# DoHoonKim8/halo2-lasso

Hardware: AMD Instinct MI355X
Metric: lasso_prove_time_ms (lower is better)
Workload: dtype u256 (BN254 Fr/Fq, 8x u32 Montgomery); 1 GPU; 2^24 AND Lasso lookup (32-bit operands, 4 chunks of 8+8 bits); lookups_per_proof=16777216, pcs=multilinear KZG (BN254), proof_bytes=64256, parallelism=1 GPU

## Files before the change

### bindings/rust/src/sys.rs

```rust
#![allow(non_camel_case_types, dead_code)]
use halo2_curves::bn256::{Fr, G1Affine, G2Affine};
use std::os::raw::{c_char, c_int, c_void};

pub type lh_status = c_int;
pub const LH_OK: lh_status = 0;
pub const LH_ERR_INVALID_SUMCHECK: lh_status = -1;
pub const LH_ERR_INVALID_PCS_PARAM: lh_status = -2;
pub const LH_ERR_INVALID_PCS_OPEN: lh_status = -3;
pub const LH_ERR_INVALID_SNARK: lh_status = -4;
pub const LH_ERR_SERIALIZATION: lh_status = -5;
pub const LH_ERR_TRANSCRIPT: lh_status = -6;
pub const LH_ERR_DEVICE: lh_status = -7;
pub const LH_ERR_ARG: lh_status = -8;

pub const LH_SC_MAX_TERMS: usize = 48;
pub const LH_SC_MAX_FACTORS: usize = 4;
pub const LH_SC_EVALUATIONS: c_int = 0;
pub const LH_SC_COEFFICIENTS: c_int = 1;
pub const LH_LASSO_MAX_CHUNKS: usize = 8;
pub const LH_LASSO_MAX_MEMORIES: usize = 16;
pub const LH_LASSO_MAX_TERMS: usize = 16;
pub const LH_RCCL_UNIQUE_ID_BYTES: usize = 128;

#[repr(C)] pub struct lh_ctx { _p: [u8; 0] }
// ... 159 lines not shown

#[repr(C)]
#[derive(Clone, Copy, Debug, Default)]
pub struct lh_lasso_route {
    pub open_small_depth: u32,
    pub open_small_passes: u32,
    pub eq_factored_rounds: u32,
    pub standard_rounds: u32,
    pub rw_leaf_rounds: u32,
    pub resident_tails: u32,
    pub resident_rounds: u32,
    pub packed_ts_pairs: u32,
    pub derived_commitments: u32,
    pub sorted_dim_reuse: u32,
    pub sharded_rounds: u32,
    pub shard_exchanges: u32,
    pub window_table_jobs: u32,
    pub open_precommit: u32,
    pub resident_layers: u32,
    pub pp_folds: u32,
    pub msm_half_batches: u32,
    pub open_shared_sums: u32,
    pub open_precommit_staged: u32,
    pub reserved: [u32; 5],
}

extern "C" {
    pub fn lh_last_error() -> *const c_char;
    pub fn lh_version() -> *const c_char;
    pub fn lh_ctx_create(device_id: c_int, out: *mut *mut lh_ctx) -> lh_status;
    pub fn lh_ctx_destroy(ctx: *mut lh_ctx);
    pub fn lh_ctx_sync(ctx: *mut lh_ctx) -> lh_status;
    pub fn lh_ctx_stream(ctx: *mut lh_ctx) -> *mut c_void;
    pub fn lh_alloc(ctx: *mut lh_ctx, bytes: usize, d_out: *mut *mut c_void) -> lh_status;
    pub fn lh_free(ctx: *mut lh_ctx, d_ptr: *mut c_void) -> lh_status;
    pub fn lh_upload(ctx: *mut lh_ctx, d_dst: *mut c_void, src: *const c_void, bytes: usize) -> lh_status;
    pub fn lh_download(ctx: *mut lh_ctx, dst: *mut c_void, d_src: *const c_void, bytes: usize) -> lh_status;
    pub fn lh_fr_from_u64(ctx: *mut lh_ctx, d_in: *const u64, n: usize, d_out: *mut Fr) -> lh_status;
    pub fn lh_fr_from_u32(ctx: *mut lh_ctx, d_in: *const u32, n: usize, d_out: *mut Fr) -> lh_status;
    pub fn lh_fr_batch_invert(ctx: *mut lh_ctx, d_in: *const Fr, n: usize, d_out: *mut Fr) -> lh_status;
    pub fn lh_fix_var(ctx: *mut lh_ctx, d_in: *const Fr, n_in: usize, x: *const Fr, d_out: *mut Fr) -> lh_status;
    pub fn lh_eq_xy(ctx: *mut lh_ctx, y: *const Fr, num_vars: usize, d_out: *mut Fr) -> lh_status;
    pub fn lh_evaluate(ctx: *mut lh_ctx, d_polys: *const *const Fr, num_polys: usize, num_vars: usize,
                       point: *const Fr, out_evals: *mut Fr) -> lh_status;
    pub fn lh_lincomb(ctx: *mut lh_ctx, d_polys: *const *const Fr, w: *const Fr, num_polys: usize, n: usize,
                      d_out: *mut Fr) -> lh_status;
    pub fn lh_sumcheck_prove(ctx: *mut lh_ctx, prover_kind: c_int, num_vars: usize, expr: *const lh_sop,
// ... 61 lines not shown
                                      t: *mut lh_transcript) -> lh_status;
    pub fn lh_hyperplonk_verify(vp: *const lh_mkzg_vp, hvp: *const lh_hp_vparam, instances: *const *const Fr,
                                t: *mut lh_transcript) -> lh_status;
    pub fn lh_hyperplonk_verify_phases(vp: *const lh_mkzg_vp, hvp: *const lh_hp_vparam, num_phases: usize,
                                       num_witness_polys: *const usize, num_challenges: *const usize,
                                       instances: *const *const Fr, t: *mut lh_transcript) -> lh_status;
    pub fn lh_hyperplonk_prove_phases_zeromorph(ctx: *mut lh_ctx, srs: *const core::ffi::c_void, poly_size: usize,
                                                pp: *const lh_hp_param, num_phases: usize,
                                                num_witness_polys: *const usize, num_challenges: *const usize,
                                                instances: *const *const Fr, circuit: *const lh_hp_circuit,
                                                t: *mut lh_transcript) -> lh_status;
    pub fn lh_hyperplonk_verify_phases_zeromorph(vp: *const core::ffi::c_void, hvp: *const lh_hp_vparam, num_phases: usize,
                                                 num_witness_polys: *const usize, num_challenges: *const usize,
                                                 instances: *const *const Fr, t: *mut lh_transcript) -> lh_status;
    pub fn lh_debug_jit_source(code: *const u32, num_instrs: usize, num_regs: u32, result_reg: u32, degree: i32,
                               out: *mut core::ffi::c_char, cap: usize, len: *mut usize) -> lh_status;
    pub fn lh_debug_sort_pairs(ctx: *mut lh_ctx, key_bytes: i32, slabs: *const lh_debug_sort_slab, count: usize) -> lh_status;
    pub fn lh_debug_lasso_counters(ctx: *mut lh_ctx, d_dims: *const *const u32, num_cols: usize, n: usize, m: usize,
                                   d_read_ts: *const *mut u32, d_final_cts: *const *mut u32,
                                   d_keep_sorted: *const *mut u32, d_keep_index: *const *mut u32) -> lh_status;
    pub fn lh_debug_sort_plan(n: usize, bits: u32, key_bytes: i32, passes: *mut u32, rb: *mut u32,
                              temp_bytes: *mut usize) -> lh_status;
    pub fn lh_debug_u32_columns(ctx: *mut lh_ctx, op: i32, args: *const lh_debug_u32_args) -> lh_status;
    pub fn lh_ukzg_batch_commit(ctx: *mut lh_ctx, srs: *const c_void, poly_size: usize, d_polys: *const *const Fr,
                                lens: *const usize, num_polys: usize, out_comms: *mut G1Affine) -> lh_status;
    pub fn lh_ukzg_open(ctx: *mut lh_ctx, srs: *const c_void, poly_size: usize, d_poly: *const Fr, len: usize,
                        point: *const Fr, t: *mut lh_transcript) -> lh_status;
    pub fn lh_ukzg_batch_open(ctx: *mut lh_ctx, srs: *const c_void, poly_size: usize, d_polys: *const *const Fr,
                              lens: *const usize, num_polys: usize, points: *const Fr, num_points: usize,
                              evals: *const lh_evaluation, num_evals: usize, t: *mut lh_transcript) -> lh_status;
    pub fn lh_ukzg_vp_setup(s: *const Fr, out: *mut *mut c_void) -> lh_status;
    pub fn lh_ukzg_vp_free(vp: *mut c_void);
    pub fn lh_ukzg_verify(vp: *const c_void, comm: *const G1Affine, point: *const Fr, eval: *const Fr,
                          t: *mut lh_transcript) -> lh_status;
    pub fn lh_ukzg_batch_verify(vp: *const c_void, comms: *const G1Affine, num_comms: usize, points: *const Fr,
                                num_points: usize, evals: *const lh_evaluation, num_evals: usize,
                                t: *mut lh_transcript) -> lh_status;
    pub fn lh_gemini_batch_commit(ctx: *mut lh_ctx, srs: *const c_void, poly_size: usize, d_polys: *const *const Fr,
                                  num_polys: usize, num_vars: usize, out_comms: *mut G1Affine) -> lh_status;
    pub fn lh_gemini_open(ctx: *mut lh_ctx, srs: *const c_void, poly_size: usize, d_poly: *const Fr, num_vars: usize,
                          point: *const Fr, t: *mut lh_transcript) -> lh_status;
    pub fn lh_gemini_batch_open(ctx: *mut lh_ctx, srs: *const c_void, poly_size: usize, num_vars: usize,
                                d_polys: *const *const Fr, num_polys: usize, points: *const Fr, num_points: usize,
                                evals: *const lh_evaluation, num_evals: usize, t: *mut lh_transcript) -> lh_status;
    pub fn lh_gemini_verify(vp: *const c_void, comm: *const G1Affine, point: *const Fr, num_vars: usize, eval: *const Fr,
                            t: *mut lh_transcript) -> lh_status;
// ... 142 lines not shown
```

### halo2-lasso_amd/__init__.py

```python
import ctypes as C

from . import _ffi
from ._ffi import (lh_fr, lh_g1, lh_sop, lh_evaluation, lh_lasso_table, lh_transcript,
                   LH_SC_EVALUATIONS, LH_SC_COEFFICIENTS)

R_MOD = 0x30644E72E131A029B85045B68181585D2833E84879B9709143E1F593F0000001
Q_MOD = 0x30644E72E131A029B85045B68181585D97816A916871CA8D3C208C16D87CFD47
_MONT = 1 << 256
_MONT_INV_R = pow(_MONT, -1, R_MOD)
_MONT_INV_Q = pow(_MONT, -1, Q_MOD)

SUBTABLE_IDENTITY, SUBTABLE_AND, SUBTABLE_XOR = 0, 1, 2
SUBTABLE_OR, SUBTABLE_EQ, SUBTABLE_LTU = 3, 4, 5


class Error(Exception):
    code = None


class InvalidSumcheck(Error):
    code = _ffi.LH_ERR_INVALID_SUMCHECK


class InvalidPcsParam(Error):
# ... 1386 lines not shown
    n_local = (1 << poly.num_vars) >> rho
    out = poly.ctx.alloc(32 * n_local)
    _check(poly.ctx.lib.lh_shard_extract(poly.ctx.h, poly.ptr, n_local, shard_bit, rho, rank, 32, out.ptr))
    return MultilinearPolynomial(poly.ctx, out, poly.num_vars - rho)


def lasso_prove_sharded(pp, table, num_vars, dims_local, transcript):
    if len(dims_local) != table.c:
        raise ArgumentError("expected %d dim columns" % table.c)
    t = table.to_c()
    _check(pp.ctx.lib.lh_lasso_prove_sharded(pp.ctx.h, pp.h, C.byref(t), num_vars, _ptr_array(dims_local), transcript.p))


def lasso_last_timing(ctx):
    out = (C.c_double * _ffi.LH_LASSO_NUM_PHASES)()
    _check(ctx.lib.lh_lasso_last_timing(ctx.h, out))
    names = ["witness", "commit", "surge", "leaves", "gkr", "evals", "open_n", "open_l", "total"]
    return dict(zip(names, list(out)))


ROUTE_FIELDS = ["open_small_depth", "open_small_passes", "eq_factored_rounds", "standard_rounds", "rw_leaf_rounds",
                "resident_tails", "resident_rounds", "packed_ts_pairs", "derived_commitments", "sorted_dim_reuse",
                "sharded_rounds", "shard_exchanges", "window_table_jobs", "open_precommit", "resident_layers", "pp_folds", "msm_half_batches",
                "open_shared_sums", "open_precommit_staged"]


def lasso_last_route(ctx):
    out = (C.c_uint32 * 24)()
    _check(ctx.lib.lh_lasso_last_route(ctx.h, out))
    return dict(zip(ROUTE_FIELDS, [int(v) for v in out]))


def set_option(ctx, name, value):
    _check(ctx.lib.lh_ctx_set_option(ctx.h, name.encode(), int(value)))


def get_option(ctx, name):
    out = C.c_int64(0)
    _check(ctx.lib.lh_ctx_get_option(ctx.h, name.encode(), C.byref(out)))
    return int(out.value)


def profile_enable(ctx, on=True):
    _check(ctx.lib.lh_profile_enable(ctx.h, int(on)))


def profile_read(ctx):
# ... 9 lines not shown
```

### halo2-lasso_amd/_ffi.py

```python
import ctypes as C
import os

_HERE = os.path.dirname(os.path.abspath(__file__))
LIB_PATH = os.path.join(_HERE, "liblasso_hip.so")

LH_OK = 0
LH_ERR_INVALID_SUMCHECK, LH_ERR_INVALID_PCS_PARAM, LH_ERR_INVALID_PCS_OPEN = -1, -2, -3
LH_ERR_INVALID_SNARK, LH_ERR_SERIALIZATION, LH_ERR_TRANSCRIPT, LH_ERR_DEVICE, LH_ERR_ARG = -4, -5, -6, -7, -8
LH_SC_EVALUATIONS, LH_SC_COEFFICIENTS = 0, 1
LH_SC_MAX_TERMS, LH_SC_MAX_FACTORS = 48, 4
LH_LASSO_MAX_CHUNKS, LH_LASSO_MAX_MEMORIES, LH_LASSO_MAX_TERMS = 8, 16, 16
LH_SUBTABLE_IDENTITY, LH_SUBTABLE_AND, LH_SUBTABLE_XOR, LH_SUBTABLE_OR, LH_SUBTABLE_EQ, LH_SUBTABLE_LTU = 0, 1, 2, 3, 4, 5
LH_LASSO_NUM_PHASES = 9
LH_BD_COLUMN_FR, LH_BD_COLUMN_U32 = 0, 1


class lh_fr(C.Structure):
    _fields_ = [("l", C.c_uint64 * 4)]


class lh_g1(C.Structure):
    _fields_ = [("x", C.c_uint64 * 4), ("y", C.c_uint64 * 4)]


# ... 258 lines not shown
                                      C.POINTER(lh_evaluation), _SZ, C.POINTER(lh_transcript)]),
    "lh_g1_axpy": (C.c_int, [_P, _P, _P, _SZ, C.POINTER(lh_fr), _P]),
    "lh_g1_rows_msm": (C.c_int, [_P, _P, C.c_int, C.c_uint32, _SZ, _SZ, _P, C.POINTER(lh_g1)]),
    "lh_hyrax_setup": (C.c_int, [_P, _SZ, _SZ, C.POINTER(_P)]),
    "lh_hyrax_dims": (C.c_int, [_SZ, _SZ, C.POINTER(_SZ), C.POINTER(_SZ), C.POINTER(_SZ)]),
    "lh_hyrax_trim": (C.c_int, [_P, _SZ, _SZ, C.POINTER(_SZ), C.POINTER(_SZ)]),
    "lh_hyrax_batch_commit": (C.c_int, [_P, _P, _SZ, _SZ, C.POINTER(_P), _SZ, _SZ, C.POINTER(lh_g1)]),
    "lh_hyrax_open": (C.c_int, [_P, _P, _SZ, _SZ, _P, _SZ, C.POINTER(lh_fr), C.POINTER(lh_transcript)]),
    "lh_hyrax_batch_open": (C.c_int, [_P, _P, _SZ, _SZ, _SZ, C.POINTER(_P), _SZ, C.POINTER(lh_fr), _SZ,
                                      C.POINTER(lh_evaluation), _SZ, C.POINTER(lh_transcript)]),
    "lh_hyrax_verify": (C.c_int, [_P, _SZ, _SZ, C.POINTER(lh_g1), C.POINTER(lh_fr), _SZ, C.POINTER(lh_fr),
                                  C.POINTER(lh_transcript)]),
    "lh_hyrax_batch_verify": (C.c_int, [_P, _SZ, _SZ, _SZ, C.POINTER(lh_g1), _SZ, C.POINTER(lh_fr), _SZ,
                                        C.POINTER(lh_evaluation), _SZ, C.POINTER(lh_transcript)]),
    "lh_debug_jit_source": (C.c_int, [C.POINTER(C.c_uint32), _SZ, C.c_uint32, C.c_uint32, C.c_int, C.c_char_p, _SZ,
                                      C.POINTER(_SZ)]),
    "lh_debug_sort_pairs": (C.c_int, [_P, C.c_int, C.POINTER(lh_debug_sort_slab), _SZ]),
    "lh_debug_lasso_counters": (C.c_int, [_P, C.POINTER(_P), _SZ, _SZ, _SZ, C.POINTER(_P), C.POINTER(_P), C.POINTER(_P),
                                          C.POINTER(_P)]),
    "lh_debug_sort_plan": (C.c_int, [_SZ, C.c_uint, C.c_int, C.POINTER(C.c_uint), C.POINTER(C.c_uint), C.POINTER(_SZ)]),
    "lh_debug_msm_plan": (C.c_int, [_SZ, C.POINTER(_SZ), C.POINTER(C.c_uint32), C.POINTER(C.c_uint32), C.c_int, C.c_int,
                                    C.POINTER(C.c_uint64), C.POINTER(_SZ)]),
    "lh_debug_u32_columns": (C.c_int, [_P, C.c_int, C.POINTER(lh_debug_u32_args)]),
    "lh_keccak_transcript_hash_io": (C.c_int, [C.POINTER(lh_transcript), C.POINTER(lh_hash_transcript)]),
    "lh_brakedown_setup": (C.c_int, [_P, _SZ, C.c_int, C.c_char_p, C.POINTER(_P)]),
    "lh_brakedown_derive": (C.c_int, [_SZ, C.c_int, C.POINTER(_P)]),
    "lh_brakedown_param_info": (C.c_int, [_P, C.POINTER(_SZ), C.POINTER(_SZ), C.POINTER(_SZ), C.POINTER(_SZ),
                                          C.POINTER(_SZ)]),
    "lh_brakedown_trim": (C.c_int, [_P, _SZ]),
    "lh_brakedown_param_free": (None, [_P]),
    "lh_brakedown_encode": (C.c_int, [_P, C.POINTER(lh_fr), C.POINTER(lh_fr)]),
    "lh_brakedown_commit": (C.c_int, [_P, _P, _P, _SZ, C.POINTER(_P)]),
    "lh_brakedown_batch_commit": (C.c_int, [_P, _P, C.POINTER(_P), _SZ, _SZ, C.POINTER(_P)]),
    "lh_brakedown_commit_columns": (C.c_int, [_P, _P, C.POINTER(_P), C.POINTER(C.c_int), C.POINTER(_SZ), _SZ, C.POINTER(_P)]),
    "lh_brakedown_comm_root": (C.c_int, [_P, C.c_char_p]),
    "lh_brakedown_comm_rows": (C.c_int, [_P, _P, _P]),
    "lh_brakedown_comm_rows_device": (C.c_int, [_P, C.POINTER(_P)]),
    "lh_brakedown_comm_tree": (C.c_int, [_P, _P, C.c_char_p]),
    "lh_brakedown_comm_stage": (C.c_int, [_P, _P, _P, _P]),
    "lh_brakedown_comm_free": (None, [_P]),
    "lh_hyperplonk_prove_brakedown": (C.c_int, [_P, _P, C.POINTER(lh_hp_param), C.POINTER(_P), C.POINTER(_P),
                                                C.POINTER(C.POINTER(lh_fr)), C.POINTER(_P), C.POINTER(lh_transcript),
                                                C.POINTER(lh_hash_transcript)]),
    "lh_hyperplonk_prove_phases_brakedown": (C.c_int, [_P, _P, C.POINTER(lh_hp_param), C.POINTER(_P), C.POINTER(_P), _SZ,
                                                       C.POINTER(_SZ), C.POINTER(_SZ), C.POINTER(C.POINTER(lh_fr)),
                                                       C.POINTER(lh_hp_circuit), C.POINTER(lh_transcript),
# ... 67 lines not shown
```

### halo2-lasso_amd/csrc/capi.cpp

```cpp
#include "host.hpp"
#include "brakedown.hpp"
#include <memory>

using namespace lh;

struct lh_ctx {
  Ctx c;
};
struct lh_srs {
  Srs s;
};
struct lh_mkzg_vp {
  VerifierParams* p;
};
struct lh_usrs {
  USrs s;
};
struct lh_zm_vp {
  ZmVerifierParams* p;
};
struct lh_ukzg_vp {
  UkzgVerifierParams* p;
};
struct lh_ipa_param {
// ... 2119 lines not shown
    case LH_U32_QUAD_SUMS: k_quad_sums(c, cols, a->lens, a->count, dw, a->n, (Fr*)a->d_out); break;
    case LH_U32_LINCOMB_MIXED:
      k_lincomb_mixed(c, (const Fr* const*)a->d_fr, (const Fr*)a->w_fr, a->num_fr, cols, a->lens, (const Fr*)a->w, a->count, a->n,
                      (Fr*)a->d_out);
      break;
    case LH_U32_LINCOMB_FOLD_SMALL:
      *a->taken = k_lincomb_fold_small(c, cols, a->lens, (const Fr*)a->w, a->count, a->n, r0, (Fr*)a->d_out) ? 1 : 0;
      break;
    default: {
      Fr* two = (Fr*)c.pin(65536) + 1024;
      if (op == LH_U32_LINCOMB_BIND2) {
        k_lincomb_bind2(c, cols, a->lens, (const Fr*)a->w, a->count, r0, r1, dw, a->n, (Fr*)a->d_out, two);
        memcpy(a->out_host, two, 64);
      } else {
        k_sc_round_u32_bind2(c, cols[0], dw, r0, r1, a->n, (Fr*)a->d_out, two);
        memcpy(a->out_host, two, 32);
      }
    }
  }
  c.sync();
  LH_CATCH
}

lh_status lh_profile_enable(lh_ctx* ctx, int on) {
  LH_TRY NEED_CTX(ctx);
  ctx->c.sync();
  ctx->c.prof = on == 1;
  ctx->c.prof_recs.clear();
  std::vector<ProfRec> drop;
  ctx->c.live_resolve(drop);
  ctx->c.live = on == 2;
  if (ctx->c.helper) {
    ctx->c.helper->live_resolve(drop);
    ctx->c.helper->live = on == 2;
  }
  LH_CATCH
}
lh_status lh_profile_read(lh_ctx* ctx, lh_prof_rec* out, size_t cap, size_t* count) {
  LH_TRY NEED_CTX(ctx);
  NEED(count);
  static_assert(sizeof(lh_prof_rec) == sizeof(lh::ProfRec), "profile record layout");
  if (ctx->c.live) {
    ctx->c.live_resolve(ctx->c.prof_recs);
    if (ctx->c.helper) {
      LH_HIP(hipStreamSynchronize(ctx->c.helper->stream));
      ctx->c.helper->live_resolve(ctx->c.prof_recs);
// ... 10 lines not shown
```

### halo2-lasso_amd/csrc/dev.cpp

```cpp
#include <string.h>
#include <stdlib.h>
#include <ctype.h>
#include <errno.h>
#include <sched.h>
#include <atomic>
#include <condition_variable>
#include <mutex>
#include <thread>
#include <functional>
#include <memory>
#include <emmintrin.h>
#include <hip/hip_ext.h>
#include <vector>
#include <chrono>
#include "dev.hpp"

namespace lh {

static thread_local std::string g_last_error;
void set_last_error(const char* msg) { g_last_error = msg ? msg : ""; }
const char* get_last_error() { return g_last_error.c_str(); }

Arena::~Arena() {
  for (auto& b : blocks_) (void)hipFree(b.p);
// ... 107 lines not shown
  KnobKind kind;
  double dflt, lo, hi;
  bool live;
  const char* word;
} KNOB_TABLE[] = {
    {"LH_SC_TAIL_G", INT, 0, 0, 1024},
    {"LH_MSM_C_OFF", INT, 4, -32, 32},
    {"LH_MSM_C_MAX", INT, 17, 1, 31},
    {"LH_MSM_K2", INT, 4, 2, 64},
    {"LH_MSM_SEG", INT, 0, 0, 256},
    {"LH_MSM_SLAB_LOG", INT, 16, 0, 31},
    {"LH_MSM_TREE_MAX", INT, 262144, 0, 1 << 30},
    {"LH_MSM_QUAD_MAX", INT, 262144, 0, 1 << 30},
    {"LH_MSM_TWO_LEVEL", INT, 1, 0, 1},
    {"LH_MSM_HALF_MIN_LOG", INT, 24, 0, 63},
    {"LH_MSM_HALF_COVER", INT, 12, 0, 1 << 20},
    {"LH_EXPR_MONOMIALS", INT, 0, 0, 1},
    {"LH_EXPR_JIT_MIN_VARS", INT, 16, 0, 64},
    {"LH_EXPR_EF_MIN_VARS", INT, 14, 2, 64},
    {"LH_FIN_LANES_MIN_BYTES", REAL, 0, -1, 1e18},
    {"LH_SC_U32", INT, 1, 0, 1}, {"LH_OPEN_U32_ROUNDS", INT, 1, 0, 1}, {"LH_OPEN_FOLD_COLS", INT, 1, 0, 1},
    {"LH_OPEN_SHARE_SUMS", INT, 1, 0, 1, true},
    {"LH_LASSO_PRODUCT_U32", INT, 0, 0, 1, true},
    {"LH_HOST_THREADS", INT, 48, 0, 4096},
    {"LH_JIT_CACHE", INT, 1, 0, 1}, {"LH_JIT_CACHE_DIR", PATH, 0, 0, 0},
    {"LH_EXPR_JIT", INT, 1, 0, 1},
    {"LH_SC_TAIL_TIMEOUT_MS", REAL, 2000, 0, 1e7, true}, {"LH_GKR_START_TIMEOUT_MS", REAL, 25, 0, 1e7, true},
    {"LH_COMM_WAIT_TIMEOUT_MS", INT, 30000, 1, 1e9}, {"LH_COMM_A2A", WORD, 0, 0, 1, false, "allgather"},
    {"LH_COMM_PROBE", INT, 1, 0, 1},
    {"LH_HOST_TRACE", INT, 0, 0, 1, true}, {"LH_SC_TAIL_TRACE", INT, 0, 0, 1}, {"LH_GKR_TRACE", INT, 0, 0, 1},
    {"LH_SC_DEBUG", INT, 0, 0, 1}, {"LH_MSM_DEBUG", INT, 0, 0, 1}, {"LH_HP_DEBUG", INT, 0, 0, 1}, {"LH_COMM_DEBUG", INT, 0, 0, 1},
    {"LH_OPEN_SMALL_CHECK", INT, 0, 0, 1},
    {"LH_COMM_A2A_SELF", INT, 0, 0, 1}, {"LH_COMM_PROBE_FAIL", INT, 0, 0, 1}, {"LH_SHARDED_COUNTERS_MIN_R", INT, 2, 1, 1 << 20},
    {"LH_TEST_PRECOMMIT_GATE", INT, 0, 0, 2, true},
};
static_assert(sizeof(KNOB_TABLE) / sizeof(KNOB_TABLE[0]) == (size_t)Knob::COUNT, "KNOB_TABLE: one row per Knob");

static double knob_read(const KnobRow& r, std::atomic<bool>* said) {
  double v = r.dflt;
  if (r.kind != WORD) {
    env_number(r.env, r.kind == REAL, r.lo, r.hi, v, said);
  } else if (const char* e = getenv(r.env)) {
    if (strcmp(e, r.word) == 0) v = 1;
    else if (*e && (!said || !said->exchange(true))) fprintf(stderr, "[lasso-hip] %s=%s is outside [%s]: ignored\n", r.env, e, r.word);
  }
  return v;
// ... 413 lines not shown
```

### halo2-lasso_amd/csrc/dev.hpp

```cpp
#pragma once
#include <hip/hip_runtime_api.h>
#include <stdint.h>
#include <stdarg.h>
#include <stdio.h>
#include <functional>
#include <memory>
#include <string>
#include <vector>
#include <utility>
#include <stdexcept>

#include "../../include/lasso_hip.h"
#include "ec.cuh"

namespace lh {

struct Error : std::exception {
  int code;
  std::string msg;
  Error(int c, std::string m) : code(c), msg(std::move(m)) {}
  const char* what() const noexcept override { return msg.c_str(); }
};

void set_last_error(const char* msg);
// ... 76 lines not shown
  int64_t lasso_pack_ts = 1;
  int64_t sc_tail = 1;
  int64_t sc_tail_max_len = 8192;
  int64_t shard_exchange_log = 19;
  int64_t open_precommit = 1;
  int64_t open_precommit_stages = 1;
  int64_t msm_window_tables = 0;
  int64_t sc_pp_fold = 1;
  int64_t msm_half_batches = 1;
  int64_t gkr_resident = 1;
  int64_t comm_round = 0;
  int64_t hyrax_rows = 1;
  int64_t brakedown_batch_commit = 1;
  int64_t brakedown_staged_open = 0;
  int64_t brakedown_u32_gather = 1;
  Options();
  int64_t* find(const char* name);
  static bool in_range(const char* name, int64_t value);
};

enum class Knob {
  SC_TAIL_G, MSM_C_OFF, MSM_C_MAX, MSM_K2, MSM_SEG, MSM_SLAB_LOG, MSM_TREE_MAX, MSM_QUAD_MAX, MSM_TWO_LEVEL, MSM_HALF_MIN_LOG,
  MSM_HALF_COVER, EXPR_MONOMIALS, EXPR_JIT_MIN_VARS, EXPR_EF_MIN_VARS,
  FIN_LANES_MIN_BYTES, SC_U32, OPEN_U32_ROUNDS, OPEN_FOLD_COLS, OPEN_SHARE_SUMS, LASSO_PRODUCT_U32,
  HOST_THREADS, JIT_CACHE, JIT_CACHE_DIR, EXPR_JIT, SC_TAIL_TIMEOUT_MS, GKR_START_TIMEOUT_MS, COMM_WAIT_TIMEOUT_MS, COMM_A2A,
  COMM_PROBE,
  HOST_TRACE, SC_TAIL_TRACE, GKR_TRACE, SC_DEBUG, MSM_DEBUG, HP_DEBUG, COMM_DEBUG, OPEN_SMALL_CHECK,
  COMM_A2A_SELF, COMM_PROBE_FAIL, SHARDED_COUNTERS_MIN_R, TEST_PRECOMMIT_GATE,
  COUNT
};
double knob(Knob k);
const char* knob_text(Knob k);
struct RouteStats {
  uint32_t v[LH_LASSO_ROUTE_WORDS] = {0};
  enum { OPEN_DEPTH, OPEN_PASSES, EF_ROUNDS, STD_ROUNDS, RW_ROUNDS, TAILS, TAIL_ROUNDS, PACKED_TS, DERIVED, SORTED_REUSE,
         SHARDED_ROUNDS, SHARD_EXCHANGES, WIN_TABLE_JOBS, OPEN_PRECOMMIT, RESIDENT_LAYERS, PP_FOLDS, MSM_HALF_BATCHES,
         OPEN_SHARED_SUMS, OPEN_PRECOMMIT_STAGED };
};

class HostWorker {
 public:
  HostWorker();
  ~HostWorker();
  void submit(std::function<void()> fn);
  void wait();
 private:
  struct Impl;
  Impl* impl_;
};

struct OpenPrecommit;
struct Ctx {
  Options opt;
  RouteStats route;
  int device = 0;
  hipStream_t stream = nullptr;
  Arena arena;
  void* pinned = nullptr;
  size_t pinned_bytes = 0;
  int num_cus = 256;
// ... 156 lines not shown
    LH_HIP(hipEventRecord(c.prof_ev[0], c.stream));
  }
  ~ProfScope() {
    if (!on) return;
    (void)hipEventRecord(c.prof_ev[1], c.stream);
    (void)hipEventSynchronize(c.prof_ev[1]);
    float ms = 0;
    (void)hipEventElapsedTime(&ms, c.prof_ev[0], c.prof_ev[1]);
    rec.ms = ms;
    c.prof_recs.push_back(rec);
  }
};

void k_fr_from_u64(Ctx&, const uint64_t* in, size_t n, Fr* out);
void k_fr_from_u32(Ctx&, const uint32_t* in, size_t n, Fr* out);
void k_fr_to_repr(Ctx&, const Fr* in, size_t n, Fr* out);
void k_fr_from_repr(Ctx&, const Fr* in, size_t n, Fr* out);
void k_fr_binop(Ctx&, int op, const Fr* a, const Fr* b, size_t n, Fr* out);
void k_fr_mul_chain(Ctx&, const Fr* a, const Fr* b, size_t n, int iters, Fr* out);
void k_fr_batch_invert(Ctx&, const Fr* in, size_t n, Fr* out);
void k_fix_var(Ctx&, const Fr* in, size_t n_in, const Fr& x, Fr* out);
void k_fix_var_multi(Ctx&, const Fr* const* in, Fr* const* out, size_t count, size_t n_in, const Fr& x);
void k_eq_xy(Ctx&, const Fr* y, size_t num_vars, Fr* out);
void k_bind_first(Ctx&, const Fr* const* in, size_t count, const Fr& x, Fr* out_host);
void k_gather_heads(Ctx&, const Fr* const* in, size_t count, int k, Fr* out_host);
void k_lincomb(Ctx&, const Fr* const* polys, const Fr* w, size_t count, size_t n, Fr* out);
void k_lincomb_fold(Ctx&, const Fr* const* polys, const Fr* w, size_t count, size_t half, const Fr& x, Fr* out);
bool k_lincomb_fold_small(Ctx&, const uint32_t* const* cols, const size_t* lens, const Fr* coef, size_t count, size_t half,
                          const Fr& x, Fr* out);
void k_inner_products(Ctx&, const Fr* const* polys, size_t count, const Fr* weights, size_t n, Fr* out_host);
constexpr int LCM_MAX_FR = 8, LCM_MAX_SMALL = 24;
constexpr int LCF_MAX = 24;
constexpr int LCB_MAX = 24;
void k_inner_products_small(Ctx&, const uint32_t* const* polys, size_t count, const Fr* weights, size_t n, Fr* out_host);
void k_inner_products_small_half(Ctx&, const uint32_t* const* polys, size_t count, const Fr* eq_half, size_t half,
                                 const Fr& y0, Fr* out_host);
void k_inner_products_small_quads(Ctx&, const uint32_t* col, const Fr* e0, size_t quads, Fr* out_host);
void k_inner_products_quads(Ctx&, const uint32_t* const* cols, const size_t* lens, size_t count, const Fr* e1, size_t quads,
                            Fr* d_out);
constexpr int QS_MAX_COLS = 24;
void k_quad_sums(Ctx&, const uint32_t* const* cols, const size_t* lens, size_t count, const Fr* e0, size_t quads, Fr* d_out);
void k_lincomb_bind2(Ctx&, const uint32_t* const* cols, const size_t* lens, const Fr* w, size_t count, const Fr& r0, const Fr& r1,
                     const Fr* eq_level, size_t size, Fr* out, Fr* out_host);
void k_sc_round_u32_bind2(Ctx&, const uint32_t* col, const Fr* eq_level, const Fr& r0, const Fr& r1, size_t size, Fr* out,
                          Fr* out_host);
void k_lincomb_mixed(Ctx&, const Fr* const* fr, const Fr* wfr, size_t num_fr, const uint32_t* const* sm,
// ... 326 lines not shown
```

### halo2-lasso_amd/csrc/expr.cpp

```cpp
#include <algorithm>
#include <map>
#include "host.hpp"
#include "expr.hpp"

namespace lh {

static const uint32_t BH_PRIMITIVES[32] = {
    1, 3, 7, 11, 19, 37, 67, 131, 285, 529, 1033, 2053, 4179, 8219, 16427, 32771, 65581, 131081, 262183, 524327,
    1048585, 2097157, 4194307, 8388641, 16777243, 33554441, 67108935, 134217767, 268435465, 536870917, 1073741907,
    2147483657u};
static const uint32_t BH_X_INVS[32] = {
    0, 1, 3, 5, 9, 18, 33, 65, 142, 264, 516, 1026, 2089, 4109, 8213, 16385, 32790, 65540, 131091, 262163, 524292,
    1048578, 2097153, 4194320, 8388621, 16777220, 33554467, 67108883, 134217732, 268435458, 536870953, 1073741828};

uint32_t bh_primitive(size_t num_vars) { return BH_PRIMITIVES[num_vars]; }
uint32_t bh_x_inv(size_t num_vars) { return BH_X_INVS[num_vars]; }
size_t bh_next(size_t b, size_t num_vars) {
  b <<= 1;
  return b ^ ((b >> num_vars) * BH_PRIMITIVES[num_vars]);
}
size_t bh_nth(size_t num_vars, size_t i) {
  if (i == 0) return 0;
  size_t b = 1;
  for (size_t k = 1; k < i; k++) b = bh_next(b, num_vars);
// ... 518 lines not shown
        {
          std::vector<HFr> d(num_vars), pre(num_vars + 1);
          pre[0] = HFr::one();
          for (size_t i = 0; i < num_vars; i++) d[i] = HFr::one() - y[i], pre[i + 1] = pre[i] * d[i];
          HFr inv = pre[num_vars].inv();
          ef.inv_1my.resize(num_vars);
          for (size_t i = num_vars; i-- > 0;) {
            ef.inv_1my[i] = inv * pre[i];
            inv = inv * d[i];
          }
        }
        ef.per_term = false, ef.trusted_claim = false;
        ef.kappa = shp.kappa;
        const HFr kappa_inv = shp.kappa.inv();
        ef.c = sum * kappa_inv;
        EqFactoring::One one;
        one.table = t_eq, one.y = y, one.S = one.S_prev = HFr::one();
        {
          const size_t half = n >> 1;
          Fr* buf = c.arena.alloc_n<Fr>(2 * half);
          one.level.resize(num_vars);
          size_t off = 0;
          for (size_t jl = 0; jl < num_vars; jl++) one.level[jl] = buf + off, off += half >> jl;
          k_eq_xy(c, (const Fr*)(y + 1), num_vars - 1, buf);
          std::vector<Fr*> lower;
          for (size_t jl = 1; jl < num_vars; jl++) lower.push_back((Fr*)one.level[jl]);
          k_eq_levels(c, one.level[0], half, lower.data(), lower.size());
        }
        ef.eqs.push_back(one);
        ef.streams = [](bool, size_t) { return true; };
        LinSums ls;
        memset(&ls, 0, sizeof(ls));
        ls.count = (uint32_t)shp.lin.size();
        for (uint32_t i = 0; i < ls.count; i++) ls.coeff[i] = dev(shp.lin[i].second);
        ef.round = [&](const Fr* const* in, Fr* const* out, const Fr& r, bool bind, size_t size, size_t round, int points,
                       Fr* out_host) {
          ArenaScope round_scope(c.arena);
          if (bind) {
            std::vector<const Fr*> src;
            std::vector<Fr*> dst;
            for (size_t i = 0; i < T; i++)
              if (used[i] && i != t_eq) src.push_back(in[i]), dst.push_back(out[i]);
            k_fix_var_multi(c, src.data(), dst.data(), src.size(), 4 * size, r);
          }
          for (size_t i = 0; i < T; i++) prc.in[i] = bind ? out[i] : in[i];
          prc.in[t_eq] = ef.eqs[0].level[round];
          if (ls.count) {
            for (uint32_t i = 0; i < ls.count; i++) ls.t[i] = prc.in[table_of[shp.lin[i].first]];
            k_lin_sums(c, ls, size, out_host + 12);
          }
// ... 29 lines not shown
```

### halo2-lasso_amd/csrc/kernels_poly.hip

```cpp
#include <hip/hip_runtime.h>
#include <string.h>
#include <algorithm>
#include "dev.hpp"
#include "ff_host.hpp"
#include "reduce.cuh"
#include "resident.cuh"
#include "wide.cuh"

namespace lh {

static inline dim3 grid_for(size_t n, int block = 256, size_t cap = 4096) {
  size_t g = (n + block - 1) / block;
  if (g < 1) g = 1;
  if (g > cap) g = cap;
  return dim3((unsigned)g);
}
#define GSTRIDE(i, n) \
  for (size_t i = (size_t)blockIdx.x * blockDim.x + threadIdx.x; i < (n); i += (size_t)gridDim.x * blockDim.x)

__global__ void fr_from_u64_kernel(const uint64_t* __restrict__ in, size_t n, Fr* __restrict__ out) {
  GSTRIDE(i, n) out[i] = from_u64<FrParams>(in[i]);
}
__global__ void fr_from_u32_kernel(const uint32_t* __restrict__ in, size_t n, Fr* __restrict__ out) {
  GSTRIDE(i, n) out[i] = from_u64<FrParams>(in[i]);
// ... 216 lines not shown
  EqGroups g;
  size_t first[EQ_GROUPS], cnt[EQ_GROUPS];
  Fr* tab[EQ_GROUPS];
  for (size_t k = 0, done = 0; k < ngroups; k++) {
    cnt[k] = (num_vars - done + (ngroups - k) - 1) / (ngroups - k);
    first[k] = done;
    done += cnt[k];
    tab[k] = ngroups == 1 ? out : c.arena.alloc_n<Fr>((size_t)1 << cnt[k]);
    g.levels[k] = (int)cnt[k];
    g.out[k] = tab[k];
    for (size_t i = 0; i < cnt[k]; i++) g.y[k][i] = y[first[k] + cnt[k] - 1 - i];
  }
  hipLaunchKernelGGL(eq_groups_kernel, dim3((unsigned)ngroups), dim3(256), 0, c.stream, g);
  Fr* cur = tab[0];
  size_t done = cnt[0];
  for (size_t k = 1; k < ngroups; k++) {
    const bool last = k + 1 == ngroups;
    const size_t n = (size_t)1 << (done + cnt[k]);
    Fr* dst = last ? out : c.arena.alloc_n<Fr>(n);
    hipLaunchKernelGGL(eq_outer_kernel, grid_for(n), 256, 0, c.stream, cur, (int)done, tab[k], n, dst);
    cur = dst;
    done += cnt[k];
  }
}

template <class T>
__global__ void shard_extract_kernel(const T* __restrict__ g, size_t n_local, unsigned j, unsigned rho, size_t s,
                                     T* __restrict__ local) {
  const size_t lo_mask = ((size_t)1 << j) - 1;
  GSTRIDE(i, n_local) local[i] = g[((i >> j) << (j + rho)) | (s << j) | (i & lo_mask)];
}
struct alignas(16) Bytes64 {
  uint4 a, b, c, d;
};
void k_shard_extract(Ctx& c, const void* global, size_t n_local, size_t j, size_t rho, size_t s, size_t elem,
                     void* local) {
  if (!n_local) return;
  dim3 g = grid_for(n_local);
  if (elem == 4)
    hipLaunchKernelGGL(shard_extract_kernel<uint32_t>, g, 256, 0, c.stream, (const uint32_t*)global, n_local, (unsigned)j,
                       (unsigned)rho, s, (uint32_t*)local);
  else if (elem == 32)
    hipLaunchKernelGGL(shard_extract_kernel<Fr>, g, 256, 0, c.stream, (const Fr*)global, n_local, (unsigned)j,
                       (unsigned)rho, s, (Fr*)local);
  else if (elem == 64)
    hipLaunchKernelGGL(shard_extract_kernel<Bytes64>, g, 256, 0, c.stream, (const Bytes64*)global, n_local, (unsigned)j,
// ... 1312 lines not shown
```

### halo2-lasso_amd/csrc/sumcheck.cpp

```cpp
#include <algorithm>
#include <functional>
#include <chrono>
#include <memory>
#include <thread>
#include "host.hpp"
#include "resident_host.hpp"

namespace lh {

std::vector<HFr> host_eq_xy(const std::vector<HFr>& y) {
  if (y.empty()) return {};
  std::vector<HFr> evals{HFr::one()};
  for (size_t i = y.size(); i-- > 0;) {
    std::vector<HFr> nxt(evals.size() * 2);
    for (size_t k = 0; k < evals.size(); k++) {
      nxt[2 * k + 1] = evals[k] * y[i];
      nxt[2 * k] = evals[k] - nxt[2 * k + 1];
    }
    evals.swap(nxt);
  }
  return evals;
}

HFr host_eq_xy_eval(const HFr* x, const HFr* y, size_t n) {
// ... 713 lines not shown
      for (size_t b = 0; b < num_polys; b++) {
        const ScU32Terms::Poly& pl = u32t.polys[b];
        k_lincomb_mixed(c, nullptr, nullptr, 0, pl.col.data(), pl.len.data(), pl.w.data(), pl.col.size(), len0, const_cast<Fr*>(d_polys[b]));
      }
  }
  const bool pp_shape = use_ef && !ef.per_term && pp_terms;
  std::vector<HFr> pp_folded;
  bool rw_folded = false;
  if (use_ef) {
    const Shard shg(c);
    const size_t half = (size_t)1 << (nvl - 1);
    for (EqFactoring::One& one : ef.eqs) {
      const Fr* shared = eq_half_lookup(c, one.y, num_vars, sharded);
      Fr* buf = c.arena.alloc_n<Fr>(shared ? half : 2 * half);
      one.level.resize(num_vars);
      size_t off = 0;
      for (size_t jl = 0; jl < nvl; jl++) {
        if (jl == 0 && shared) {
          one.level[0] = const_cast<Fr*>(shared);
          continue;
        }
        one.level[jl] = buf + off;
        off += half >> jl;
      }
      if (!shared) {
        if (sharded) eq_xy_shard(c, shg, one.y, num_vars, 1, buf);
        else k_eq_xy(c, (const Fr*)(one.y + 1), num_vars - 1, buf);
      }
      std::vector<Fr*> lower;
      for (size_t jl = 1; jl < nvl; jl++) lower.push_back((Fr*)one.level[jl]);
      k_eq_levels(c, one.level[0], half, lower.data(), lower.size());
    }
    ef.streams = [&](bool, size_t size) { return k_sc_round_streams(rd, degree, size); };
    ef.round = [&](const Fr* const* in, Fr* const* out, const Fr& r, bool bind, size_t size, size_t round, int points,
                   Fr* out_host) {
      if (!ef.per_term && rw && rw_folded) {
        LH_REQUIRE(points == 2, LH_ERR_ARG, "sum-check: tree-pair rounds asked for an extra point after the fold");
        ScRound g;
        memset(&g, 0, sizeof(g));
        g.num_tables = 2 * rw->num_pairs, g.num_terms = rw->num_pairs;
        for (size_t i = 0; i < 2 * (size_t)rw->num_pairs; i++) g.in[i] = in[i], g.out[i] = out[i];
        for (uint32_t m = 0; m < rw->num_pairs; m++) {
          g.coeff[m] = dev(HFr::one()), g.coeff_is_one[m] = 1;
          g.nfac[m] = 2, g.fac[m][0] = (uint8_t)(2 * m), g.fac[m][1] = (uint8_t)(2 * m + 1);
        }
        g.r = r;
// ... 233 lines not shown
```

### include/lasso_hip.h

```cpp
#ifndef LASSO_HIP_H
#define LASSO_HIP_H

#include <stddef.h>
#include <stdint.h>

#ifdef __cplusplus
extern "C" {
#endif

typedef struct { uint64_t l[4]; } lh_fr;
typedef struct { uint64_t x[4], y[4]; } lh_g1;

typedef int lh_status;
#define LH_OK 0
#define LH_ERR_INVALID_SUMCHECK (-1)
#define LH_ERR_INVALID_PCS_PARAM (-2)
#define LH_ERR_INVALID_PCS_OPEN (-3)
#define LH_ERR_INVALID_SNARK (-4)
#define LH_ERR_SERIALIZATION (-5)
#define LH_ERR_TRANSCRIPT (-6)
#define LH_ERR_DEVICE (-7)
#define LH_ERR_ARG (-8)

typedef struct lh_ctx lh_ctx;
// ... 136 lines not shown
lh_status lh_ctx_set_option(lh_ctx*, const char* name, int64_t value);
lh_status lh_ctx_get_option(lh_ctx*, const char* name, int64_t* out);
#define LH_LASSO_ROUTE_WORDS 24
typedef struct lh_lasso_route {
  uint32_t open_small_depth;
  uint32_t open_small_passes;
  uint32_t eq_factored_rounds;
  uint32_t standard_rounds;
  uint32_t rw_leaf_rounds;
  uint32_t resident_tails;
  uint32_t resident_rounds;
  uint32_t packed_ts_pairs;
  uint32_t derived_commitments;
  uint32_t sorted_dim_reuse;
  uint32_t sharded_rounds;
  uint32_t shard_exchanges;
  uint32_t window_table_jobs;
  uint32_t open_precommit;
  uint32_t resident_layers;
  uint32_t pp_folds;
  uint32_t msm_half_batches;
  uint32_t open_shared_sums;
  uint32_t open_precommit_staged;
  uint32_t reserved[5];
} lh_lasso_route;
lh_status lh_lasso_last_route(lh_ctx*, lh_lasso_route* out);

typedef struct lh_comm {
  int rank, size;
  void* user;
  int (*all_gather)(void* user, const void* send, void* recv, size_t bytes_per_rank);
  int (*all_gather_device)(void* user, const void* d_send, void* d_recv, size_t bytes_per_rank, void* hip_stream);
} lh_comm;
lh_status lh_ctx_set_comm(lh_ctx*, const lh_comm* comm, size_t shard_bit);
#define LH_RCCL_UNIQUE_ID_BYTES 128
lh_status lh_rccl_unique_id(uint8_t out[LH_RCCL_UNIQUE_ID_BYTES]);
lh_status lh_ctx_set_comm_rccl(lh_ctx*, int rank, int size, const uint8_t unique_id[LH_RCCL_UNIQUE_ID_BYTES],
                               size_t shard_bit);
lh_status lh_ctx_set_comm_loopback(lh_ctx*, int rank, int size, size_t shard_bit);
lh_status lh_ctx_comm_stats(lh_ctx*, uint64_t out[2]);
lh_status lh_ctx_comm_phase_stats(lh_ctx*, uint64_t out[16], int reset);
lh_status lh_ctx_memory_stats(lh_ctx*, uint64_t out[4]);
lh_status lh_ctx_compute_units(lh_ctx*, size_t* out);
lh_status lh_ctx_host_cpus(lh_ctx*, char* bus_id, size_t bus_id_cap, char* cpulist, size_t cpulist_cap);
lh_status lh_lasso_prove_sharded(lh_ctx*, const lh_srs*, const lh_lasso_table*, size_t num_vars,
                                 const uint32_t* const* d_dims_local, lh_transcript* t);

// ... 319 lines not shown
  LH_U32_LINCOMB_MIXED = 4,
  LH_U32_LINCOMB_FOLD_SMALL = 5,
  LH_U32_LINCOMB_BIND2 = 6,
  LH_U32_SC_ROUND_BIND2 = 7,
  LH_U32_QUAD_SUMS = 9
};
typedef struct lh_debug_u32_args {
  const uint32_t* const* d_cols;
  const size_t* lens;
  const lh_fr* w;
  size_t count;
  const lh_fr* d_weights;
  size_t n;
  const lh_fr* const* d_fr;
  const lh_fr* w_fr;
  size_t num_fr;
  lh_fr r0, r1;
  lh_fr* d_out;
  lh_fr* out_host;
  int* taken;
} lh_debug_u32_args;
lh_status lh_debug_u32_columns(lh_ctx*, int op, const lh_debug_u32_args*);

typedef struct lh_prof_rec {
  char name[40];
  double ms;
  double bytes;
  double muls;
  double items;
} lh_prof_rec;
lh_status lh_profile_enable(lh_ctx*, int on);
lh_status lh_profile_read(lh_ctx*, lh_prof_rec* out, size_t cap, size_t* count);

#ifdef __cplusplus
}
#endif
#endif
```

Measured before the change: 53.08 ms.

## Fuse eq table and all level tables into one kernel launch

Adds a single kernel that writes the eq(x,y) table and every lower-level partial eq table in one launch. It builds a shared-memory tree for the low 8 variables, gives each block per-row coefficients for the high variables, and uses extra blocks for the small upper levels. This replaces the separate k_eq_xy plus k_eq_levels passes in the sumcheck and expression eq-factored paths, avoiding the launch overhead and the re-read of the top level. In exchange, redundant multiplications are done per row and per upper-level entry.

```diff
diff --git a/bindings/rust/src/sys.rs b/bindings/rust/src/sys.rs
--- a/bindings/rust/src/sys.rs
+++ b/bindings/rust/src/sys.rs
@@ -205,7 +205,8 @@
     pub msm_half_batches: u32,
     pub open_shared_sums: u32,
     pub open_precommit_staged: u32,
-    pub reserved: [u32; 5],
+    pub eq_fused_launches: u32,
+    pub reserved: [u32; 4],
 }
 
 extern "C" {
@@ -313,6 +314,7 @@
     pub fn lh_debug_sort_plan(n: usize, bits: u32, key_bytes: i32, passes: *mut u32, rb: *mut u32,
                               temp_bytes: *mut usize) -> lh_status;
     pub fn lh_debug_u32_columns(ctx: *mut lh_ctx, op: i32, args: *const lh_debug_u32_args) -> lh_status;
+    pub fn lh_debug_eq_fused(ctx: *mut lh_ctx, y: *const lh_fr, num_vars: usize, d_levels: *const *mut lh_fr) -> lh_status;
     pub fn lh_ukzg_batch_commit(ctx: *mut lh_ctx, srs: *const c_void, poly_size: usize, d_polys: *const *const Fr,
                                 lens: *const usize, num_polys: usize, out_comms: *mut G1Affine) -> lh_status;
     pub fn lh_ukzg_open(ctx: *mut lh_ctx, srs: *const c_void, poly_size: usize, d_poly: *const Fr, len: usize,
diff --git a/halo2-lasso_amd/__init__.py b/halo2-lasso_amd/__init__.py
--- a/halo2-lasso_amd/__init__.py
+++ b/halo2-lasso_amd/__init__.py
@@ -1432,7 +1432,7 @@
 ROUTE_FIELDS = ["open_small_depth", "open_small_passes", "eq_factored_rounds", "standard_rounds", "rw_leaf_rounds",
                 "resident_tails", "resident_rounds", "packed_ts_pairs", "derived_commitments", "sorted_dim_reuse",
                 "sharded_rounds", "shard_exchanges", "window_table_jobs", "open_precommit", "resident_layers", "pp_folds", "msm_half_batches",
-                "open_shared_sums", "open_precommit_staged"]
+                "open_shared_sums", "open_precommit_staged", "eq_fused_launches"]
 
 
 def lasso_last_route(ctx):
diff --git a/halo2-lasso_amd/_ffi.py b/halo2-lasso_amd/_ffi.py
--- a/halo2-lasso_amd/_ffi.py
+++ b/halo2-lasso_amd/_ffi.py
@@ -304,6 +304,7 @@
     "lh_debug_msm_plan": (C.c_int, [_SZ, C.POINTER(_SZ), C.POINTER(C.c_uint32), C.POINTER(C.c_uint32), C.c_int, C.c_int,
                                     C.POINTER(C.c_uint64), C.POINTER(_SZ)]),
     "lh_debug_u32_columns": (C.c_int, [_P, C.c_int, C.POINTER(lh_debug_u32_args)]),
+    "lh_debug_eq_fused": (C.c_int, [_P, C.POINTER(lh_fr), _SZ, C.POINTER(_P)]),
     "lh_keccak_transcript_hash_io": (C.c_int, [C.POINTER(lh_transcript), C.POINTER(lh_hash_transcript)]),
     "lh_brakedown_setup": (C.c_int, [_P, _SZ, C.c_int, C.c_char_p, C.POINTER(_P)]),
     "lh_brakedown_derive": (C.c_int, [_SZ, C.c_int, C.POINTER(_P)]),
diff --git a/halo2-lasso_amd/csrc/capi.cpp b/halo2-lasso_amd/csrc/capi.cpp
--- a/halo2-lasso_amd/csrc/capi.cpp
+++ b/halo2-lasso_amd/csrc/capi.cpp
@@ -2165,6 +2165,18 @@
   LH_CATCH
 }
 
+lh_status lh_debug_eq_fused(lh_ctx* ctx, const lh_fr* y, size_t num_vars, lh_fr* const* d_levels) {
+  LH_TRY NEED_CTX(ctx);
+  NEED_N(y, num_vars);
+  NEED(d_levels);
+  LH_REQUIRE(k_eq_fused_takes(num_vars), LH_ERR_ARG, "debug eq fused: too many variables");
+  std::vector<Fr> yv(num_vars);
+  if (num_vars) memcpy(yv.data(), y, num_vars * sizeof(Fr));
+  k_eq_fused(ctx->c, yv.data(), num_vars, (Fr* const*)d_levels);
+  ctx->c.sync();
+  LH_CATCH
+}
+
 lh_status lh_profile_enable(lh_ctx* ctx, int on) {
   LH_TRY NEED_CTX(ctx);
   ctx->c.sync();
diff --git a/halo2-lasso_amd/csrc/dev.cpp b/halo2-lasso_amd/csrc/dev.cpp
--- a/halo2-lasso_amd/csrc/dev.cpp
+++ b/halo2-lasso_amd/csrc/dev.cpp
@@ -153,6 +153,7 @@
     {"LH_SC_U32", INT, 1, 0, 1}, {"LH_OPEN_U32_ROUNDS", INT, 1, 0, 1}, {"LH_OPEN_FOLD_COLS", INT, 1, 0, 1},
     {"LH_OPEN_SHARE_SUMS", INT, 1, 0, 1, true},
     {"LH_LASSO_PRODUCT_U32", INT, 0, 0, 1, true},
+    {"LH_EQ_FUSED", INT, 1, 0, 1, true},
     {"LH_HOST_THREADS", INT, 48, 0, 4096},
     {"LH_JIT_CACHE", INT, 1, 0, 1}, {"LH_JIT_CACHE_DIR", PATH, 0, 0, 0},
     {"LH_EXPR_JIT", INT, 1, 0, 1},
diff --git a/halo2-lasso_amd/csrc/dev.hpp b/halo2-lasso_amd/csrc/dev.hpp
--- a/halo2-lasso_amd/csrc/dev.hpp
+++ b/halo2-lasso_amd/csrc/dev.hpp
@@ -122,7 +122,7 @@
 enum class Knob {
   SC_TAIL_G, MSM_C_OFF, MSM_C_MAX, MSM_K2, MSM_SEG, MSM_SLAB_LOG, MSM_TREE_MAX, MSM_QUAD_MAX, MSM_TWO_LEVEL, MSM_HALF_MIN_LOG,
   MSM_HALF_COVER, EXPR_MONOMIALS, EXPR_JIT_MIN_VARS, EXPR_EF_MIN_VARS,
-  FIN_LANES_MIN_BYTES, SC_U32, OPEN_U32_ROUNDS, OPEN_FOLD_COLS, OPEN_SHARE_SUMS, LASSO_PRODUCT_U32,
+  FIN_LANES_MIN_BYTES, SC_U32, OPEN_U32_ROUNDS, OPEN_FOLD_COLS, OPEN_SHARE_SUMS, LASSO_PRODUCT_U32, EQ_FUSED,
   HOST_THREADS, JIT_CACHE, JIT_CACHE_DIR, EXPR_JIT, SC_TAIL_TIMEOUT_MS, GKR_START_TIMEOUT_MS, COMM_WAIT_TIMEOUT_MS, COMM_A2A,
   COMM_PROBE,
   HOST_TRACE, SC_TAIL_TRACE, GKR_TRACE, SC_DEBUG, MSM_DEBUG, HP_DEBUG, COMM_DEBUG, OPEN_SMALL_CHECK,
@@ -135,7 +135,7 @@
   uint32_t v[LH_LASSO_ROUTE_WORDS] = {0};
   enum { OPEN_DEPTH, OPEN_PASSES, EF_ROUNDS, STD_ROUNDS, RW_ROUNDS, TAILS, TAIL_ROUNDS, PACKED_TS, DERIVED, SORTED_REUSE,
          SHARDED_ROUNDS, SHARD_EXCHANGES, WIN_TABLE_JOBS, OPEN_PRECOMMIT, RESIDENT_LAYERS, PP_FOLDS, MSM_HALF_BATCHES,
-         OPEN_SHARED_SUMS, OPEN_PRECOMMIT_STAGED };
+         OPEN_SHARED_SUMS, OPEN_PRECOMMIT_STAGED, EQ_FUSED };
 };
 
 class HostWorker {
@@ -338,6 +338,8 @@
 void k_fix_var(Ctx&, const Fr* in, size_t n_in, const Fr& x, Fr* out);
 void k_fix_var_multi(Ctx&, const Fr* const* in, Fr* const* out, size_t count, size_t n_in, const Fr& x);
 void k_eq_xy(Ctx&, const Fr* y, size_t num_vars, Fr* out);
+bool k_eq_fused_takes(size_t num_vars);
+void k_eq_fused(Ctx&, const Fr* y, size_t num_vars, Fr* const* level);
 void k_bind_first(Ctx&, const Fr* const* in, size_t count, const Fr& x, Fr* out_host);
 void k_gather_heads(Ctx&, const Fr* const* in, size_t count, int k, Fr* out_host);
 void k_lincomb(Ctx&, const Fr* const* polys, const Fr* w, size_t count, size_t n, Fr* out);
diff --git a/halo2-lasso_amd/csrc/expr.cpp b/halo2-lasso_amd/csrc/expr.cpp
--- a/halo2-lasso_amd/csrc/expr.cpp
+++ b/halo2-lasso_amd/csrc/expr.cpp
@@ -564,10 +564,16 @@
           one.level.resize(num_vars);
           size_t off = 0;
           for (size_t jl = 0; jl < num_vars; jl++) one.level[jl] = buf + off, off += half >> jl;
-          k_eq_xy(c, (const Fr*)(y + 1), num_vars - 1, buf);
-          std::vector<Fr*> lower;
-          for (size_t jl = 1; jl < num_vars; jl++) lower.push_back((Fr*)one.level[jl]);
-          k_eq_levels(c, one.level[0], half, lower.data(), lower.size());
+          if (knob(Knob::EQ_FUSED) != 0 && k_eq_fused_takes(num_vars - 1)) {
+            std::vector<Fr*> all;
+            for (size_t jl = 0; jl < num_vars; jl++) all.push_back((Fr*)one.level[jl]);
+            k_eq_fused(c, (const Fr*)(y + 1), num_vars - 1, all.data());
+          } else {
+            k_eq_xy(c, (const Fr*)(y + 1), num_vars - 1, buf);
+            std::vector<Fr*> lower;
+            for (size_t jl = 1; jl < num_vars; jl++) lower.push_back((Fr*)one.level[jl]);
+            k_eq_levels(c, one.level[0], half, lower.data(), lower.size());
+          }
         }
         ef.eqs.push_back(one);
         ef.streams = [](bool, size_t) { return true; };
diff --git a/halo2-lasso_amd/csrc/kernels_poly.hip b/halo2-lasso_amd/csrc/kernels_poly.hip
--- a/halo2-lasso_amd/csrc/kernels_poly.hip
+++ b/halo2-lasso_amd/csrc/kernels_poly.hip
@@ -262,6 +262,89 @@
     cur = dst;
     done += cnt[k];
   }
+}
+
+constexpr int EQF_LO = 8, EQF_MAX_VARS = 30, EQF_MAX_ROWS = 16, EQF_THREADS = 256;
+struct EqFused {
+  Fr y[EQF_MAX_VARS];
+  Fr* level[EQF_MAX_VARS + 1];
+  uint32_t m, lo, rows, main_blocks;
+};
+__global__ __launch_bounds__(EQF_THREADS) void eq_fused_kernel(EqFused g) {
+  __shared__ Fr heap[2 << EQF_LO];
+  __shared__ Fr coef[EQF_MAX_ROWS];
+  __shared__ Fr* lv[EQF_MAX_VARS + 1];
+  const uint32_t m = g.m, L = g.lo, tid = threadIdx.x;
+  if (tid == 0)
+    for (uint32_t j = 0; j <= m; j++) lv[j] = g.level[j];
+  if (blockIdx.x >= g.main_blocks) {
+    __syncthreads();
+    const size_t f = (size_t)(blockIdx.x - g.main_blocks) * EQF_THREADS + tid + 1;
+    if (f >= ((size_t)1 << (m - L))) return;
+    const uint32_t k = 63 - __clzll((unsigned long long)f), j = m - k;
+    const size_t b = f - ((size_t)1 << k);
+    Fr* dst = lv[j];
+    if (!dst) return;
+    Fr acc = Fr::one();
+    for (uint32_t i = L + 1; i < m; i++) {
+      const Fr yi = g.y[i];
+      if (i >= j) acc = mul(acc, (b >> (i - j)) & 1 ? yi : sub(Fr::one(), yi));
+    }
+    dst[b] = acc;
+    return;
+  }
+  const uint32_t rows = g.rows;
+  const size_t u0 = (size_t)blockIdx.x * rows;
+  if (tid == 0) heap[1] = Fr::one();
+  if (tid >= EQF_THREADS - rows) {
+    const uint32_t r = tid - (EQF_THREADS - rows);
+    const size_t u = u0 + r;
+    Fr acc = Fr::one();
+    for (uint32_t i = L; i < m; i++) {
+      const Fr yi = g.y[i];
+      acc = mul(acc, (u >> (i - L)) & 1 ? yi : sub(Fr::one(), yi));
+    }
+    coef[r] = acc;
+  }
+  __syncthreads();
+  for (uint32_t s = 0; s < L; s++) {
+    const Fr ys = g.y[L - 1 - s];
+    if (tid < (1u << s)) {
+      const Fr e = heap[(1u << s) + tid], hi = mul(e, ys);
+      heap[(2u << s) + 2 * tid + 1] = hi;
+      heap[(2u << s) + 2 * tid] = sub(e, hi);
+    }
+    __syncthreads();
+  }
+  const uint32_t per = 2u << L, total = rows * per;
+  for (uint32_t o = tid; o < total; o += EQF_THREADS) {
+    const uint32_t r = o >> (L + 1), t = o & (per - 1);
+    if (!t) continue;
+    const uint32_t i = 31 - __clz(t);
+    Fr* dst = lv[L - i];
+    if (dst) dst[((u0 + r) << i) | (t - (1u << i))] = mul(coef[r], heap[t]);
+  }
+}
+bool k_eq_fused_takes(size_t num_vars) { return num_vars <= (size_t)EQF_MAX_VARS; }
+void k_eq_fused(Ctx& c, const Fr* y, size_t num_vars, Fr* const* level) {
+  LH_REQUIRE(k_eq_fused_takes(num_vars), LH_ERR_ARG, "eq_fused: too many variables");
+  double entries = 0;
+  EqFused g;
+  memset(&g, 0, sizeof(g));
+  for (size_t j = 0; j <= num_vars; j++) {
+    if (j < num_vars) g.y[j] = y[j];
+    g.level[j] = level[j];
+    if (level[j]) entries += (double)((size_t)1 << (num_vars - j));
+  }
+  ProfScope ps(c, "eq_fused", 32.0 * entries, entries, entries);
+  c.route.v[RouteStats::EQ_FUSED]++;
+  g.m = (uint32_t)num_vars;
+  g.lo = (uint32_t)std::min<size_t>(num_vars, EQF_LO);
+  const size_t upper = (size_t)1 << (num_vars - g.lo);
+  g.rows = (uint32_t)std::min<size_t>(std::max<size_t>(upper >> 10, 1), EQF_MAX_ROWS);
+  g.main_blocks = (uint32_t)(upper / g.rows);
+  const size_t above = (upper - 1 + EQF_THREADS - 1) / EQF_THREADS;
+  hipLaunchKernelGGL(eq_fused_kernel, dim3((unsigned)(g.main_blocks + above)), dim3(EQF_THREADS), 0, c.stream, g);
 }
 
 template <class T>
diff --git a/halo2-lasso_amd/csrc/sumcheck.cpp b/halo2-lasso_amd/csrc/sumcheck.cpp
--- a/halo2-lasso_amd/csrc/sumcheck.cpp
+++ b/halo2-lasso_amd/csrc/sumcheck.cpp
@@ -759,6 +759,12 @@
         }
         one.level[jl] = buf + off;
         off += half >> jl;
+      }
+      if (!sharded && knob(Knob::EQ_FUSED) != 0 && k_eq_fused_takes(num_vars - 1)) {
+        std::vector<Fr*> all(num_vars);
+        for (size_t jl = 0; jl < num_vars; jl++) all[jl] = jl == 0 && shared ? nullptr : (Fr*)one.level[jl];
+        k_eq_fused(c, (const Fr*)(one.y + 1), num_vars - 1, all.data());
+        continue;
       }
       if (!shared) {
         if (sharded) eq_xy_shard(c, shg, one.y, num_vars, 1, buf);
diff --git a/include/lasso_hip.h b/include/lasso_hip.h
--- a/include/lasso_hip.h
+++ b/include/lasso_hip.h
@@ -182,7 +182,8 @@
   uint32_t msm_half_batches;
   uint32_t open_shared_sums;
   uint32_t open_precommit_staged;
-  uint32_t reserved[5];
+  uint32_t eq_fused_launches;
+  uint32_t reserved[4];
 } lh_lasso_route;
 lh_status lh_lasso_last_route(lh_ctx*, lh_lasso_route* out);
 
@@ -548,6 +549,8 @@
 } lh_debug_u32_args;
 lh_status lh_debug_u32_columns(lh_ctx*, int op, const lh_debug_u32_args*);
 
+lh_status lh_debug_eq_fused(lh_ctx*, const lh_fr* y, size_t num_vars, lh_fr* const* d_levels);
+
 typedef struct lh_prof_rec {
   char name[40];
   double ms;
```

After: 53.00 ms (median of 6 runs). Within noise of the previous version (-0.2%).
